# stcodeer/Frequency-wised_All-in-One_Image_Restoration_Model

Hardware: AMD Instinct MI355X
Metric: training images/sec @128x128 (higher is better)
Workload: dtype bf16; 1 GPU; BASELINE configs[1]: Uformer encoder+decoder (all_3_bands, L=3, freq MSA), denoise sigma=25, 128x128, phase-2 train step (fwd+bwd+Adam, DropPath on); per_gpu_batch=16, global_batch=16, parallelism=dp1, hip_graph=True

## Files before the change

frequency-wised_all-in-one_image_restoration_model_amd/csrc/fw_norm.hip:

```cpp
#include "fw_common.h"
#include <stdlib.h>

namespace {

constexpr int NVMAX = 4;

template <int G> FW_DEV float group_sum(float v) {
#pragma unroll
    for (int o = G / 2; o > 0; o >>= 1) v += __shfl_xor(v, o, 64);
    return v;
}

template <typename T> struct RawV;
template <> struct RawV<float> {
    f32x4 v;
    FW_MEM void load(const float* p) { v = *reinterpret_cast<const f32x4*>(p); }
    FW_MEM void unpack(float* f) const { f[0] = v[0]; f[1] = v[1]; f[2] = v[2]; f[3] = v[3]; }
};
template <> struct RawV<bf16raw> {
    uint2 v;
    FW_MEM void load(const bf16raw* p) { v = *reinterpret_cast<const uint2*>(p); }
    FW_MEM void unpack(float* f) const {
        f[0] = __uint_as_float(v.x << 16); f[1] = __uint_as_float(v.x & 0xffff0000u);
        f[2] = __uint_as_float(v.y << 16); f[3] = __uint_as_float(v.y & 0xffff0000u);
// ... 47 lines not shown
            s += v[u][t][0] + v[u][t][1] + v[u][t][2] + v[u][t][3];
        }
        const float mu = group_sum<G>(s) * invc;
        float q = 0.f;
#pragma unroll
        for (int t = 0; t < NV; ++t) {
            if (gl + G * t < nv) {
#pragma unroll
                for (int e = 0; e < 4; ++e) { const float d = v[u][t][e] - mu; q += d * d; }
            }
        }
        const float rs = rsqrtf(group_sum<G>(q) * invc + eps);
        if (row >= rows) continue;
        if (gl == 0) { mean[row] = mu; rstd[row] = rs; }
#pragma unroll
        for (int t = 0; t < NV; ++t) {
            const int c4 = gl + G * t;
            if (c4 < nv) {
                float o[4];
#pragma unroll
                for (int e = 0; e < 4; ++e) o[e] = (v[u][t][e] - mu) * rs * gam[t][e] + bet[t][e];
                if (MOD) {
#pragma unroll
                    for (int e = 0; e < 4; ++e) o[e] += mv[u][t][e];
                }
                T* yp = y + row * ldy + c4 * 4;
                if (sizeof(T) == 4) *reinterpret_cast<f32x4*>(yp) = f32x4{o[0], o[1], o[2], o[3]};
                else *reinterpret_cast<uint2*>(yp) = make_uint2(pack_bf2(o[0], o[1]), pack_bf2(o[2], o[3]));
            }
        }
    }
}

template <typename T, int G, int NV, int U>
__global__ __launch_bounds__(256) void ln_bwd_kernel(const T* __restrict__ dy, long lddy, const float* __restrict__ x, long ldx,
                                                     const float* __restrict__ gamma, const float* __restrict__ mean,
                                                     const float* __restrict__ rstd, const float* __restrict__ dres, long lddres,
                                                     float* __restrict__ dx, long lddx, float* __restrict__ partial,
                                                     long pstride, int rows, int C, T* __restrict__ twin, long ldtw,
                                                     const float* __restrict__ twscale, int tw_rows_per_scale) {
    constexpr int RPB = 256 / G;
    const int gl = threadIdx.x % G, gr = threadIdx.x / G;
    const int nv = C >> 2;
    const float invc = 1.0f / C;
    f32x4 gam[NV], dg[NV], db[NV];
    bool cok[NV];
#pragma unroll
    for (int t = 0; t < NV; ++t) {
        const int c4 = gl + G * t;
        cok[t] = c4 < nv;
        gam[t] = cok[t] ? *reinterpret_cast<const f32x4*>(gamma + c4 * 4) : f32x4{0.f, 0.f, 0.f, 0.f};
        dg[t] = f32x4{0.f, 0.f, 0.f, 0.f};
        db[t] = f32x4{0.f, 0.f, 0.f, 0.f};
    }
    for (long r0 = (long)blockIdx.x * RPB * U; r0 < rows; r0 += (long)gridDim.x * RPB * U) {
        f32x4 xv[U][NV], rr[U][NV];
        RawV<T> dr[U][NV];
        float mu[U], rs[U];
#pragma unroll
        for (int u = 0; u < U; ++u) {
            const long row = r0 + u * RPB + gr;
            const long rc = row < rows ? row : rows - 1;
            mu[u] = mean[rc]; rs[u] = rstd[rc];
#pragma unroll
            for (int t = 0; t < NV; ++t) {
                const int cc = (cok[t] ? gl + G * t : nv - 1) * 4;
                xv[u][t] = *reinterpret_cast<const f32x4*>(x + rc * ldx + cc);
                dr[u][t].load(dy + rc * lddy + cc);
                if (dres) rr[u][t] = *reinterpret_cast<const f32x4*>(dres + rc * lddres + cc);
            }
        }
#pragma unroll
        for (int u = 0; u < U; ++u) {
            const long row = r0 + u * RPB + gr;
            const bool live = row < rows;
            f32x4 xh[NV], g[NV];
            float s1 = 0.f, s2 = 0.f;
#pragma unroll
            for (int t = 0; t < NV; ++t) {
                float d[4];
                dr[u][t].unpack(d);
                const bool ok = live && cok[t];
#pragma unroll
                for (int e = 0; e < 4; ++e) {
                    const float de = ok ? d[e] : 0.f;
                    xh[t][e] = ok ? (xv[u][t][e] - mu[u]) * rs[u] : 0.f;
                    g[t][e] = de * gam[t][e];
                    dg[t][e] += de * xh[t][e];
                    db[t][e] += de;
                    s1 += g[t][e];
                    s2 += g[t][e] * xh[t][e];
                }
            }
            s1 = group_sum<G>(s1) * invc;
            s2 = group_sum<G>(s2) * invc;
            if (!live) continue;
            const float sc = (twin && twscale) ? twscale[row / tw_rows_per_scale] : 1.0f;
#pragma unroll
            for (int t = 0; t < NV; ++t) {
                if (!cok[t]) continue;
                const int c4 = gl + G * t;
                f32x4 o;
#pragma unroll
                for (int e = 0; e < 4; ++e) o[e] = rs[u] * (g[t][e] - s1 - xh[t][e] * s2);
                if (dres) o += rr[u][t];
                *reinterpret_cast<f32x4*>(dx + row * lddx + c4 * 4) = o;
                if (twin) {
                    T* tp = twin + row * ldtw + c4 * 4;
                    if (sizeof(T) == 4) *reinterpret_cast<f32x4*>(tp) = o * sc;
                    else *reinterpret_cast<uint2*>(tp) = make_uint2(pack_bf2(o[0] * sc, o[1] * sc), pack_bf2(o[2] * sc, o[3] * sc));
                }
            }
        }
    }
    __shared__ float red[2][1024];
    for (int i = threadIdx.x; i < 2048; i += 256) (&red[0][0])[i] = 0.f;
    __syncthreads();
#pragma unroll
    for (int t = 0; t < NV; ++t) {
        const int c4 = gl + G * t;
        if (c4 < nv) {
#pragma unroll
            for (int e = 0; e < 4; ++e) {
                atomicAdd(&red[0][c4 * 4 + e], dg[t][e]);
                atomicAdd(&red[1][c4 * 4 + e], db[t][e]);
            }
        }
    }
    __syncthreads();
    float* pp = partial + (long)blockIdx.x * pstride;
    const int Cp = (int)(pstride >> 1);
    for (int c = threadIdx.x; c < Cp; c += 256) {
        pp[c] = c < C ? red[0][c] : 0.f;
        pp[Cp + c] = c < C ? red[1][c] : 0.f;
    }
}

template <typename T, int G, int NV, int U>
int ln_fwd_launch(const float* x, long ldx, const float* g, const float* b, void* y, long ldy, float* mean,
                  float* rstd, int rows, int C, float eps, hipStream_t st) {
    const int rpb = 256 / G * U;
    hipLaunchKernelGGL((ln_fwd_kernel<T, G, NV, U>), dim3(fw_cdiv(rows, rpb)), dim3(256), 0, st, x, ldx, g, b, (T*)y, ldy,
                       mean, rstd, rows, C, eps, (const float*)nullptr, 1, 1, 0);
    FW_LAUNCH_RET();
}
template <typename T, int G, int NV, int U>
int ln_mod_fwd_launch(const float* x, long ldx, const float* g, const float* b, const float* mod, void* y, long ldy, float* mean,
                      float* rstd, int rows, int C, int H, int W, int shift, float eps, hipStream_t st) {
    const int rpb = 256 / G * U;
    hipLaunchKernelGGL((ln_fwd_kernel<T, G, NV, U, true>), dim3(fw_cdiv(rows, rpb)), dim3(256), 0, st, x, ldx, g, b, (T*)y, ldy,
                       mean, rstd, rows, C, eps, mod, H, W, shift);
    FW_LAUNCH_RET();
}
static inline int ln_group(int C) { return C <= 32 ? 8 : (C <= 64 ? 16 : (C <= 128 ? 32 : 64)); }
static inline int ln_rows_per_step(int C) { return C <= 256 ? 4 : (C <= 512 ? 2 : 1); }
static inline int ln_bwd_grid(int rows, int C) {
    const int cap = C > 256 ? 256 : (C > 128 ? 512 : 1024);
    return min(fw_cdiv(rows, 256 / ln_group(C) * ln_rows_per_step(C)), cap);
}

template <typename T, int G, int NV, int U>
int ln_bwd_launch(const void* dy, long lddy, const float* x, long ldx, const float* g, const float* mean,
                  const float* rstd, const float* dres, long lddres, float* dx, long lddx, float* partial, long pstride,
                  int rows, int C, void* twin, long ldtw, const float* twscale, int twrps, hipStream_t st) {
    hipLaunchKernelGGL((ln_bwd_kernel<T, G, NV, U>), dim3(ln_bwd_grid(rows, C)), dim3(256), 0, st, (const T*)dy, lddy, x, ldx, g, mean, rstd,
                       dres, lddres, dx, lddx, partial, pstride, rows, C, (T*)twin, ldtw, twscale, twrps);
    FW_LAUNCH_RET();
}

template <typename T, int E> struct ModV;
template <> struct ModV<float, 4> {
    f32x4 v;
    FW_MEM void load(const float* p) { v = *reinterpret_cast<const f32x4*>(p); }
    FW_MEM void add(float* a) const { a[0] += v[0]; a[1] += v[1]; a[2] += v[2]; a[3] += v[3]; }
};
template <> struct ModV<bf16raw, 4> {
    RawV<bf16raw> r;
    FW_MEM void load(const bf16raw* p) { r.load(p); }
    FW_MEM void add(float* a) const { float f[4]; r.unpack(f); a[0] += f[0]; a[1] += f[1]; a[2] += f[2]; a[3] += f[3]; }
};
template <> struct ModV<bf16raw, 8> {
    uint4 v;
    FW_MEM void load(const bf16raw* p) { v = *reinterpret_cast<const uint4*>(p); }
    FW_MEM void add(float* a) const {
        const unsigned w[4] = {v.x, v.y, v.z, v.w};
#pragma unroll
        for (int i = 0; i < 4; ++i) { a[2 * i] += __uint_as_float(w[i] << 16); a[2 * i + 1] += __uint_as_float(w[i] & 0xffff0000u); }
    }
};

constexpr int MOD_LD = 8;

template <typename T, int E, int CL>
__global__ __launch_bounds__(256) void mod_bwd_kernel(const T* __restrict__ dy, long lddy, float* __restrict__ partial, int n, int per,
                                                      int C, int W, int shift) {
    constexpr int TG = 32 / CL;
    const int cl = threadIdx.x % CL, tg = threadIdx.x / CL % TG, xq = threadIdx.x / 32;
    const int yq = blockIdx.y, z = blockIdx.z;
    const int col = (blockIdx.x * CL + cl) * E;
    const bool cok = col < C;
// ... 48 lines not shown
    hipLaunchKernelGGL((mod_bwd_kernel<T, E, CL>), dim3(fw_cdiv(nvr, CL), 8, nz), dim3(256), 0, st, (const T*)dy, lddy, partial, n, \
                       per, C, W, shift)
    if (nvr <= 8) MOD_B(8);
    else if (nvr <= 16) MOD_B(16);
    else MOD_B(32);
#undef MOD_B
    FW_LAUNCH_RET();
}

#define LN_DISPATCH(FN, T, ...)                                    \
    (C <= 32 ? FN<T, 8, 1, 4>(__VA_ARGS__)                         \
     : C <= 64 ? FN<T, 16, 1, 4>(__VA_ARGS__)                      \
     : C <= 128 ? FN<T, 32, 1, 4>(__VA_ARGS__)                     \
     : C <= 256 ? FN<T, 64, 1, 4>(__VA_ARGS__)                     \
     : C <= 512 ? FN<T, 64, 2, 2>(__VA_ARGS__)                     \
                : FN<T, 64, 4, 1>(__VA_ARGS__))

}

extern "C" int fw_layernorm_fwd(int dtype, const float* x, long ldx, const float* gamma, const float* beta, void* y,
                                long ldy, float* mean, float* rstd, int rows, int C, float eps, void* stream) {
    FW_CHECK_ARG(rows > 0 && C > 0 && C % 4 == 0 && C <= 1024 && ldx % 4 == 0 && ldy % 4 == 0);
    FW_CHECK_ARG(x && gamma && beta && y && mean && rstd);
    hipStream_t st = (hipStream_t)stream;
#define LN_F(T) LN_DISPATCH(ln_fwd_launch, T, x, ldx, gamma, beta, y, ldy, mean, rstd, rows, C, eps, st)
    return dtype == FW_DT_BF16 ? LN_F(bf16raw) : LN_F(float);
#undef LN_F
}

extern "C" int fw_layernorm_bwd_blocks(int rows, int C) { return ln_bwd_grid(rows, C); }

extern "C" int fw_slab_reduce(const float* slab, int nz, long n, long zstride, float* dst, int accumulate, float* dst2, long off2, long n2,
                              void* stream);
extern "C" int fw_layernorm_bwd2(int dtype, const void* dy, long lddy, const float* x, long ldx, const float* gamma,
                                 const float* mean, const float* rstd, const float* dres, long lddres, float* dx,
                                 long lddx, float* dgamma, float* dbeta, float* partial, int rows, int C, void* twin, long ldtw,
                                 const float* twscale, int tw_rows_per_scale, void* stream) {
    FW_CHECK_ARG(rows > 0 && C > 0 && C % 4 == 0 && C <= 1024 && ldx % 4 == 0 && lddy % 4 == 0 && lddx % 4 == 0);
    FW_CHECK_ARG(dy && x && gamma && mean && rstd && dx && partial && ((dgamma && dbeta) || (!dgamma && !dbeta)));
    FW_CHECK_ARG(!twin || (ldtw % 4 == 0 && (!twscale || tw_rows_per_scale > 0)));
    hipStream_t st = (hipStream_t)stream;
    const long pstride = 2L * C;
#define LN_B(T)                                                                                                          \
    LN_DISPATCH(ln_bwd_launch, T, dy, lddy, x, ldx, gamma, mean, rstd, dres, lddres, dx, lddx, partial, pstride, rows, C, twin, \
                ldtw, twscale, tw_rows_per_scale, st)
    const int rc = dtype == FW_DT_BF16 ? LN_B(bf16raw) : LN_B(float);
#undef LN_B
    if (rc || !dgamma) return rc;
    return fw_slab_reduce(partial, ln_bwd_grid(rows, C), C, pstride, dgamma, 1, dbeta, C, C, stream);
}

extern "C" int fw_layernorm_bwd(int dtype, const void* dy, long lddy, const float* x, long ldx, const float* gamma,
                                const float* mean, const float* rstd, const float* dres, long lddres, float* dx,
                                long lddx, float* dgamma, float* dbeta, float* partial, int rows, int C, void* stream) {
    return fw_layernorm_bwd2(dtype, dy, lddy, x, ldx, gamma, mean, rstd, dres, lddres, dx, lddx, dgamma, dbeta, partial, rows, C,
                             nullptr, 0, nullptr, 1, stream);
}

extern "C" int fw_layernorm_mod_fwd(int dtype, const float* x, long ldx, const float* gamma, const float* beta, const float* mod, void* y,
                                    long ldy, float* mean, float* rstd, int rows, int C, int H, int W, int shift, float eps, void* stream) {
    FW_CHECK_ARG(rows > 0 && C > 0 && C % 4 == 0 && C <= 1024 && ldx % 4 == 0 && ldy % 4 == 0);
    FW_CHECK_ARG(x && gamma && beta && mod && y && mean && rstd && ((uintptr_t)mod & 15) == 0);
    FW_CHECK_ARG(H > 0 && W > 0 && H % 8 == 0 && W % 8 == 0 && rows % ((long)H * W) == 0 && shift >= 0 && shift < 8);
    hipStream_t st = (hipStream_t)stream;
#define LN_F(T) LN_DISPATCH(ln_mod_fwd_launch, T, x, ldx, gamma, beta, mod, y, ldy, mean, rstd, rows, C, H, W, shift, eps, st)
    return dtype == FW_DT_BF16 ? LN_F(bf16raw) : LN_F(float);
#undef LN_F
}

extern "C" int fw_modulator_bwd_blocks(int rows, int C) { return mod_bwd_slices(rows, C); }

extern "C" int fw_modulator_bwd(int dtype, const void* dy, long lddy, float* dmod, float* partial, int rows, int C, int H, int W, int shift,
                                void* stream) {
    FW_CHECK_ARG(rows > 0 && C > 0 && C % 4 == 0 && C <= 1024 && lddy % 4 == 0 && lddy >= C);
    FW_CHECK_ARG(dy && partial && ((uintptr_t)partial & 15) == 0);
    FW_CHECK_ARG(H > 0 && W > 0 && H % 8 == 0 && W % 8 == 0 && rows % ((long)H * W) == 0 && shift >= 0 && shift < 8);
    hipStream_t st = (hipStream_t)stream;
    int rc;
    if (dtype != FW_DT_BF16) {
        FW_CHECK_ARG(((uintptr_t)dy & 15) == 0);
        rc = mod_bwd_launch<float, 4>(dy, lddy, partial, rows, C, W, shift, st);
    } else if (C % 8 == 0 && lddy % 8 == 0 && ((uintptr_t)dy & 15) == 0) {
// ... 9 lines not shown
```

frequency-wised_all-in-one_image_restoration_model_amd/fwair/functional.py:

```python
import weakref

import torch

from . import ops
from .lib import call, dt


class config:
    compute_dtype = torch.float32
    shadow_epoch = 0
    direct_grads = False


def act_empty(rows, cols, dtype, device):
    ld = (cols + 7) // 8 * 8
    return torch.empty((rows, ld), dtype=dtype, device=device)[:, :cols]


def aligned(t):
    if t.stride(1) == 1 and (t.stride(0) * t.element_size()) % 16 == 0 and t.data_ptr() % 16 == 0:
        return t
    out = act_empty(t.shape[0], t.shape[1], t.dtype, t.device)
    out.copy_(t)
    return out


_shadow = {}


def shadow(param, kind='plain'):
    dtype = config.compute_dtype
    p = param.detach()
    fs = getattr(param, '_fw_shadow', None)
    if fs is not None and kind == 'plain' and fs.dtype == dtype:
        return fs
    if kind == 'plain' and dtype == torch.float32:
        w = p.reshape(p.shape[0], -1)
        if (w.stride(0) * 4) % 16 == 0:
            return w
    slot = _shadow.get(id(param))
    ent = slot[1] if slot is not None and slot[0]() is param else None
    key = (kind, dtype)
    stamp = (param._version, config.shadow_epoch, p.data_ptr())
    if ent is not None and key in ent and ent[key][0] == stamp:
# ... 123 lines not shown
                _retired_tables.append(_refresh_tables[which])
            _refresh_tables[which] = cached
        call('fw_permute3_multi', cached[1], cached[2], cached[3], cached[4])
    for ent, key, fresh, out, recipe in stamps:
        ent[key] = (fresh, out, recipe)


def _zeros(shape, device):
    return torch.zeros(shape, dtype=torch.float32, device=device)


def _grad_target(param, shape=None):
    if config.direct_grads and param is not None and param.grad is not None:
        g = param.grad
        return (g if shape is None else g.view(shape)), None
    z = _zeros(param.shape if shape is None else shape, param.device)
    return z, z


def _wgrad(g, x, n, k, m, weight, bias=None):
    dw, rw = _grad_target(weight, (n, k))
    db, rb = _grad_target(bias) if bias is not None else (None, None)
    direct = rw is None and rb is None
    ops.wgrad(g, x, n, k, m, dw, db, defer=direct)
    return (rw.view_as(weight) if rw is not None else None), rb


def _bgrad(g, bias):
    db, rb = _grad_target(bias)
    ops.colsum(g, db)
    return rb


class LayerNormFn(torch.autograd.Function):
    @staticmethod
    def forward(ctx, x, gamma, beta):
        rows, C = x.shape
        y = act_empty(rows, C, config.compute_dtype, x.device)
        mean = torch.empty(rows, dtype=torch.float32, device=x.device)
        rstd = torch.empty(rows, dtype=torch.float32, device=x.device)
        call('fw_layernorm_fwd', dt(y.dtype), x, x.stride(0), gamma, beta, y, y.stride(0), mean, rstd, rows, C, 1e-5)
        ctx.save_for_backward(x, gamma, mean, rstd)
        ctx.beta = beta
        return y

    @staticmethod
    def backward(ctx, dy):
        x, gamma, mean, rstd = ctx.saved_tensors
        dy = aligned(dy)
        beta = ctx.beta
        dg, rg = _grad_target(gamma)
        db, rb = _grad_target(beta)
        dx = ops.layernorm_bwd(dy, x, gamma, mean, rstd, dg, db, defer=rg is None and rb is None)
        return dx, rg, rb


class LinearFn(torch.autograd.Function):

    @staticmethod
    def forward(ctx, x, weight, bias, residual, rowscale, rows_per_scale, x_pre, gelu_out, out_f32, fuse=None):
        ctx.set_materialize_grads(False)
        M, K = x.shape
        N = weight.shape[0]
        if fuse is not None and not gelu_out:
            y, g = fuse['y'], None
        elif fuse is not None:
            y, g = _leff_fused_forward(x, weight, bias, fuse)
        else:
            w = shadow(weight)
            if residual is not None or out_f32:
                y = torch.empty((M, N), dtype=torch.float32, device=x.device)
            else:
                y = act_empty(M, N, x.dtype, x.device)
            g = act_empty(M, N, x.dtype, x.device) if gelu_out else None
            ops.gemm(x, w, M, N, K, out=y, bias=bias, rowscale=rowscale, rows_per_scale=rows_per_scale, residual=residual,
                     out_gelu=g)
        ctx.save_for_backward(x, weight, rowscale, x_pre)
        ctx.bias = bias
        ctx.cfg = (rows_per_scale, residual is not None)
        if gelu_out:
            ctx.mark_non_differentiable(g)
            return y, g
        return y

    @staticmethod
    def backward(ctx, dy, *_):
        if dy is None:
            return (None,) * 10
        x, weight, rowscale, x_pre = ctx.saved_tensors
        rows_per_scale, has_res = ctx.cfg
        bias = ctx.bias
        M, K = x.shape
        N = weight.shape[0]
        tw = getattr(dy, '_fw_twin', None)
        if (tw is not None and tw[0].dtype == x.dtype and tw[0].shape == (M, N) and tw[2] == rows_per_scale
                and (tw[1] is rowscale or (tw[1] is not None and rowscale is not None and tw[1].data_ptr() == rowscale.data_ptr()))):
            g = tw[0]
        elif dy.dtype == torch.float32 and x.dtype != torch.float32 or rowscale is not None:
            g = act_empty(M, N, x.dtype, x.device)
            call('fw_cast_rows', dt(x.dtype), dy, dy.stride(0), g, g.stride(0), M, N, rowscale, rows_per_scale)
        else:
            g = aligned(dy)
        dw, db = _wgrad(g, x, N, K, M, weight, bias)
        dx = dpre = None
        if ctx.needs_input_grad[0] or (x_pre is not None and ctx.needs_input_grad[6]):
            d = act_empty(M, K, x.dtype, x.device)
            ops.dgrad(g, shadow(weight), M, K, N, d, act=2 if x_pre is not None else 0, aux=x_pre)
            if x_pre is not None:
                dpre = d
            else:
                dx = d
        return dx, dw, db, (dy if has_res else None), None, None, dpre, None, None, None


def _leff_fused_forward(xn, w1, b1, fuse):
    M, C = xn.shape
    B, H, W = fuse['geo']
    C4 = w1.shape[0]
    h1, g1 = act_empty(M, C4, xn.dtype, xn.device), act_empty(M, C4, xn.dtype, xn.device)
    h2, g2 = act_empty(M, C4, xn.dtype, xn.device), act_empty(M, C4, xn.dtype, xn.device)
    y = torch.empty((M, C), dtype=torch.float32, device=xn.device)
    res, rs = fuse['residual'], fuse['rowscale']
    call('fw_leff_fwd', xn, xn.stride(0), shadow(w1, 'leff1'), b1, shadow(fuse['wd'], 'dw9'), fuse['bd'], shadow(fuse['w2'], 'leff2'), fuse['b2'],
         res, res.stride(0), rs, fuse['rows_per_scale'], y, y.stride(0), h1, g1, h2, g2, h1.stride(0), B, H, W, C)
    fuse['h2'], fuse['g2'], fuse['y'] = h2, g2, y
    return h1, g1


class LnResFn(torch.autograd.Function):

    @staticmethod
    def forward(ctx, x, gamma, beta):
        ctx.set_materialize_grads(False)
        ctx.rs_hint = getattr(x, '_fw_rs', None)
        rows, C = x.shape
        y = act_empty(rows, C, config.compute_dtype, x.device)
        mean = torch.empty(rows, dtype=torch.float32, device=x.device)
        rstd = torch.empty(rows, dtype=torch.float32, device=x.device)
        call('fw_layernorm_fwd', dt(y.dtype), x, x.stride(0), gamma, beta, y, y.stride(0), mean, rstd, rows, C, 1e-5)
        ctx.save_for_backward(x, gamma, mean, rstd)
        ctx.beta = beta
        return x.view_as(x), y

    @staticmethod
    def backward(ctx, dres, dy):
        x, gamma, mean, rstd = ctx.saved_tensors
        dg, rg = _grad_target(gamma)
        db, rb = _grad_target(ctx.beta)
        if dy is None:
            return dres, None, None
        dy = aligned(dy)
        twin = None
        if ctx.rs_hint is not None:
            twin = act_empty(x.shape[0], x.shape[1], dy.dtype, x.device)
        rs, rps = ctx.rs_hint if ctx.rs_hint is not None else (None, 1)
        dx = ops.layernorm_bwd(dy, x, gamma, mean, rstd, dg, db, dres=dres, defer=rg is None and rb is None, twin=twin, twscale=rs,
                               tw_rows_per_scale=rps)
        if twin is not None:
            dx._fw_twin = (twin, rs, rps)
        return dx, rg, rb


class LnResModFn(torch.autograd.Function):

    @staticmethod
    def forward(ctx, x, gamma, beta, mod, geo):
        ctx.set_materialize_grads(False)
        ctx.rs_hint = getattr(x, '_fw_rs', None)
        rows, C = x.shape
        y = act_empty(rows, C, config.compute_dtype, x.device)
        mean, rstd = ops.layernorm_mod_fwd(x, gamma, beta, mod, geo[0], geo[1], geo[2], y)
        ctx.save_for_backward(x, gamma, mean, rstd)
        ctx.beta, ctx.mod, ctx.geo = beta, mod, geo
        return x.view_as(x), y

    @staticmethod
    def backward(ctx, dres, dy):
        x, gamma, mean, rstd = ctx.saved_tensors
        dg, rg = _grad_target(gamma)
        db, rb = _grad_target(ctx.beta)
        if dy is None:
            return dres, None, None, None, None
        dm, rm = _grad_target(ctx.mod)
        dy = aligned(dy)
# ... 10 lines not shown


def linear(x, weight, bias=None, residual=None, rowscale=None, rows_per_scale=1, x_pre=None, gelu_out=False, out_f32=False, fuse=None):
    y = LinearFn.apply(x, weight, bias, residual, rowscale, rows_per_scale, x_pre, gelu_out, out_f32, fuse)
    if residual is not None and y.requires_grad and (x.dtype != torch.float32 or rowscale is not None):
        y._fw_rs = (rowscale, rows_per_scale)
    return y


class QKVFn(torch.autograd.Function):

    @staticmethod
    def forward(ctx, x, wq, bq, wkv, bkv, fused):
        M, K = x.shape
        C = wq.shape[0]
        Cp = (C + 7) // 8 * 8
        buf = act_empty(M, Cp + 2 * C, x.dtype, x.device)
        if fused is not None and Cp == C:
            w3 = fused['sw'] if x.dtype == torch.bfloat16 and 'sw' in fused else (fused['w'] if x.dtype == torch.float32 else None)
        else:
            w3 = None
        ctx.cat = None
        if w3 is not None:
            ops.gemm(x, w3, M, 3 * C, K, out=buf[:, :3 * C], bias=fused['b'])
        elif Cp != C and bq is not None and bkv is not None:
            wc, bc = shadow_qkv(wq, bq, wkv, bkv)
            ops.gemm(x, wc, M, Cp + 2 * C, K, out=buf, bias=bc)
            ctx.cat = wc
        else:
            ops.gemm(x, shadow(wq), M, C, K, out=buf[:, :C], bias=bq)
            ops.gemm(x, shadow(wkv), M, 2 * C, K, out=buf[:, Cp:], bias=bkv)
        ctx.save_for_backward(x, wq, wkv)
        ctx.bq, ctx.bkv = bq, bkv
        ctx.fused = (fused, w3)
        return buf

    @staticmethod
    def backward(ctx, dbuf):
        x, wq, wkv = ctx.saved_tensors
        M, K = x.shape
        C = wq.shape[0]
        Cp = (C + 7) // 8 * 8
        dbuf = aligned(dbuf)
        fused, w3 = ctx.fused
        dx = act_empty(M, K, x.dtype, x.device)
        if w3 is not None and config.direct_grads and 'gw' in fused:
            ops.wgrad(dbuf[:, :3 * C], x, 3 * C, K, M, fused['gw'], fused['gb'], defer=True)
            ops.dgrad(dbuf[:, :3 * C], w3, M, K, 3 * C, dx)
            return dx, None, None, None, None, None
        dq, dkv = dbuf[:, :C], dbuf[:, Cp:]
        dwq, dbq = _wgrad(dq, x, C, K, M, wq, ctx.bq)
        dwkv, dbkv = _wgrad(dkv, x, 2 * C, K, M, wkv, ctx.bkv)
        if ctx.cat is not None and getattr(dbuf, '_fw_zero_pad', False):
            ops.gemm(dbuf, ctx.cat, M, K, Cp + 2 * C, w_trans=True, out=dx)
            return dx, dwq, dbq, dwkv, dbkv, None
        tmp = torch.empty((M, K), dtype=torch.float32, device=x.device)
        ops.gemm(dq, shadow(wq), M, K, C, w_trans=True, out=tmp)
        ops.gemm(dkv, shadow(wkv), M, K, 2 * C, w_trans=True, out=dx, residual=tmp)
        return dx, dwq, dbq, dwkv, dbkv, None


class WindowAttnFn(torch.autograd.Function):

    @staticmethod
    def forward(ctx, qkv, tables, coef, geo, tparam, dcoef_to):
        ctx.side = (tparam, dcoef_to)
        C, B, H, W, heads, L, mode, shift, lfs = geo
        D = C // heads
        Cp = (C + 7) // 8 * 8
        rows = qkv.shape[0]
        nkt = 1 if mode == 0 else L - 1
        out = act_empty(rows, C, qkv.dtype, qkv.device)
        lse = torch.empty((B * (H // 8) * (W // 8) * L * heads, 64), dtype=torch.float32, device=qkv.device)
        tab = ops._lfs.device_table(qkv.dtype, qkv.device) if lfs == 2 else None
        call('fw_attn_fwd', dt(qkv.dtype), D, nkt, lfs, qkv, qkv[:, Cp:], qkv[:, Cp + C:], qkv.stride(0), out, out.stride(0),
             lse, tables, coef, tab, B, H, W, heads, L, mode, shift, float(D) ** -0.5)
        ctx.save_for_backward(qkv, tables, coef, out, lse)
        ctx.geo = geo
        return out

    @staticmethod
# ... 530 lines not shown
```

frequency-wised_all-in-one_image_restoration_model_amd/fwair/ops.py:

```python
import bisect

import torch

from . import lfs as _lfs
from .lib import call, dt, lib


def _ld(t):
    assert t.dim() == 2 and t.stride(1) == 1, 'expect a row-major 2-D view'
    return t.stride(0)


def empty(rows, cols, dtype, device):
    return torch.empty((rows, cols), dtype=dtype, device=device)


def gemm(x, w, M, N, K, *, x_trans=False, w_trans=False, x_op=0, w_op=0, out=None, out_dtype=None, bias=None,
         act=0, slope=0.0, aux=None, rowscale=None, rows_per_scale=1, residual=None, accumulate=False, splitk=1,
         alpha=1.0, out_gelu=None, xsum=None, c_zstride=0, xsum_zstride=0):
    assert x.dtype == w.dtype
    if out is None:
        out = torch.empty((M, N), dtype=out_dtype or x.dtype, device=x.device)
    if accumulate:
        _note_write(out)
# ... 284 lines not shown
    host[:nprob * 16].view(nprob, 16).copy_(torch.tensor(rows, dtype=torch.int64))
    it32 = torch.tensor(items, dtype=torch.int32)
    host[nprob * 16:].view(torch.int32).view(total, 4).copy_(it32)
    table = torch.empty(host.shape, dtype=torch.int64, device=dev)
    table.copy_(host, non_blocking=True)
    probs = torch.empty(nprob * lib().fw_wgrad_group_prob_bytes(), dtype=torch.uint8, device=dev)
    _group_fire(table, probs, nprob, total, tile)
    if not torch.cuda.is_current_stream_capturing():
        for slot in _host_ring:
            if slot[0].data_ptr() == host.data_ptr():
                slot[1].record()


def wgrad(g, x, n, k, m, dw, db=None, defer=False):
    if defer and _in_backward() and _groupable(g, x, n, k, m, dw, db):
        _register_flush()
        _pending_w.append((g, x, n, k, m, dw, db))
        return
    _note_write(dw)
    _note_write(db)
    sk = pick_splitk(n, k, m, g.dtype)
    if sk == 1:
        gemm(g, x, n, k, m, x_trans=True, w_trans=True, out=dw, accumulate=True, xsum=db)
        return
    nk = (n * k + 3) // 4 * 4
    S = nk + (n + 3) // 4 * 4
    slab = torch.empty((sk, S), dtype=torch.float32, device=g.device)
    cview = slab[0, :n * k].view(n, k)
    xs = slab[0, nk:] if db is not None else None
    gemm(g, x, n, k, m, x_trans=True, w_trans=True, out=cview, splitk=sk, xsum=xs, c_zstride=S, xsum_zstride=S if db is not None else 0)
    slab_reduce(slab, sk, n * k, S, dw, db, nk, n, defer=defer)


def dgrad(g, w, M, K, N, out, act=0, aux=None):
    tiles = ((M + 127) // 128) * ((K + 127) // 128)
    sk = min(512 // max(tiles, 1), N // _DGRAD_SPLIT_ROWS) if (act == 0 and tiles < 200) else 1
    if sk <= 1:
        gemm(g, w, M, K, N, w_trans=True, out=out, act=act, aux=aux)
        return
    S = (M * K + 3) // 4 * 4
    slab = torch.empty((sk, S), dtype=torch.float32, device=g.device)
    gemm(g, w, M, K, N, w_trans=True, out=slab[0, :M * K].view(M, K), splitk=sk, c_zstride=S)
    direct = out.dtype == torch.float32 and out.is_contiguous()
    tmp = out if direct else torch.empty((M, K), dtype=torch.float32, device=g.device)
    call('fw_slab_reduce', slab, sk, M * K, S, tmp, 0, None, 0, 0)
    if not direct:
        call('fw_cast_rows', dt(out.dtype), tmp, K, out, _ld(out), M, K, None, 1)


def layernorm_fwd(x, gamma, beta, out_dtype, eps=1e-5):
    rows, C = x.shape
    y = torch.empty((rows, C), dtype=out_dtype, device=x.device)
    mean = torch.empty(rows, dtype=torch.float32, device=x.device)
    rstd = torch.empty(rows, dtype=torch.float32, device=x.device)
    call('fw_layernorm_fwd', dt(out_dtype), x, _ld(x), gamma, beta, y, _ld(y), mean, rstd, rows, C, eps)
    return y, mean, rstd


def layernorm_bwd(dy, x, gamma, mean, rstd, dgamma, dbeta, dres=None, defer=False, twin=None, twscale=None, tw_rows_per_scale=1):
    rows, C = x.shape
    dx = torch.empty((rows, C), dtype=torch.float32, device=x.device)
    nblk = lib().fw_layernorm_bwd_blocks(rows, C)
    partial = torch.empty((nblk, 2 * C), dtype=torch.float32, device=x.device)
    call('fw_layernorm_bwd2', dt(dy.dtype), dy, _ld(dy), x, _ld(x), gamma, mean, rstd, dres,
         _ld(dres) if dres is not None else 0, dx, _ld(dx), None, None, partial, rows, C,
         twin, _ld(twin) if twin is not None else 0, twscale, tw_rows_per_scale)
    slab_reduce(partial, nblk, C, 2 * C, dgamma, dbeta, C, C, defer=defer)
    return dx


def layernorm_mod_fwd(x, gamma, beta, mod, H, W, shift, y, eps=1e-5):
    rows, C = x.shape
    mean = torch.empty(rows, dtype=torch.float32, device=x.device)
    rstd = torch.empty(rows, dtype=torch.float32, device=x.device)
    call('fw_layernorm_mod_fwd', dt(y.dtype), x, _ld(x), gamma, beta, mod, y, _ld(y), mean, rstd, rows, C, H, W, shift, eps)
    return mean, rstd


def modulator_bwd(dy, dmod, H, W, shift, defer=False):
    rows, C = dy.shape
    nz = lib().fw_modulator_bwd_blocks(rows, C)
    partial = torch.empty((nz, 64 * C), dtype=torch.float32, device=dy.device)
    deferred = defer and _in_backward()
    if not deferred:
        _note_write(dmod)
    call('fw_modulator_bwd', dt(dy.dtype), dy, _ld(dy), None if deferred else dmod, partial, rows, C, H, W, shift)
    if deferred:
        slab_reduce(partial, nz, 64 * C, 64 * C, dmod, defer=True)


def attn_fwd(qkv, C, B, H, W, heads, L, mode, shift, bias, coef=None, lfs=0):
    rows = qkv.shape[0]
    D = C // heads
    nkt = 1 if mode == 0 else L - 1
    out = torch.empty((rows, C), dtype=qkv.dtype, device=qkv.device)
    nitems = B * (H // 8) * (W // 8) * L * heads
    lse = torch.empty((nitems, 64), dtype=torch.float32, device=qkv.device)
# ... 97 lines not shown
```

include/fwair.h:

```cpp
#ifndef FWAIR_H
#define FWAIR_H
#ifdef __cplusplus
extern "C" {
#endif

int fw_gemm(int dtype, const void* X, long ldx, int x_trans, int x_op, const void* W, long ldw, int w_trans, int w_op,
            void* C, long ldc, int out_f32, int accumulate, int M, int N, int K, float alpha, const float* bias, int act,
            float slope, const void* aux, long ldaux, const float* rowscale, int rows_per_scale, const float* residual,
            long ldr, int splitk, void* C2, long ldc2, float* xsum, long c_zstride, long xsum_zstride, void* stream);
int fw_gemm_last_kernel(char* buf, int n);

int fw_wgrad_group_prob_bytes(void);
int fw_wgrad_group(const void* tab, void* probs, int nprob, const void* items, int nitems, int tile, void* stream);

int fw_slab_reduce(const float* slab, int nz, long n, long zstride, float* dst, int accumulate, float* dst2, long off2, long n2,
                   void* stream);
int fw_slab_reduce_multi(const void* tab, const void* prefix, int num, long total_blocks, void* stream);

int fw_layernorm_fwd(int dtype, const float* x, long ldx, const float* gamma, const float* beta, void* y, long ldy,
                     float* mean, float* rstd, int rows, int C, float eps, void* stream);
int fw_layernorm_bwd_blocks(int rows, int C);
int fw_layernorm_bwd(int dtype, const void* dy, long lddy, const float* x, long ldx, const float* gamma, const float* mean,
                     const float* rstd, const float* dres, long lddres, float* dx, long lddx, float* dgamma, float* dbeta,
                     float* partial, int rows, int C, void* stream);
int fw_layernorm_bwd2(int dtype, const void* dy, long lddy, const float* x, long ldx, const float* gamma, const float* mean,
                      const float* rstd, const float* dres, long lddres, float* dx, long lddx, float* dgamma, float* dbeta,
                      float* partial, int rows, int C, void* twin, long ldtw, const float* twscale, int tw_rows_per_scale,
                      void* stream);

int fw_layernorm_mod_fwd(int dtype, const float* x, long ldx, const float* gamma, const float* beta, const float* mod, void* y,
                         long ldy, float* mean, float* rstd, int rows, int C, int H, int W, int shift, float eps, void* stream);
int fw_modulator_bwd_blocks(int rows, int C);
int fw_modulator_bwd(int dtype, const void* dy, long lddy, float* dmod, float* partial, int rows, int C, int H, int W, int shift,
                     void* stream);

int fw_attn_lfs_table_elems(void);
int fw_attn_fwd(int dtype, int D, int nkt, int lfs, const void* q, const void* k, const void* v, long ld, void* out, long ldo,
                float* lse, const float* bias, const float* coef, const void* lfs_tab, int B, int H, int W, int heads, int L,
                int mode, int shift, float scale, void* stream);
int fw_attn_bwd(int dtype, int D, int nkt, int lfs, const void* q, const void* k, const void* v, long ld, const void* out,
                long ldo, const void* dout, long lddo, const float* lse, const float* bias, const float* coef,
                const void* lfs_tab, void* dq, void* dk, void* dv, void* dk2, void* dv2, long ldd, float* dbias,
                float* dcoef, int B, int H, int W, int heads, int L, int mode, int shift, float scale, int dq_pad, void* stream);
int fw_attn_chunks(int dtype, int D, int nkt, int lfs, int backward, int nwin, int heads, int L);

int fw_dwconv_fwd(int dtype, const void* in, long ld1, int in_gelu, const float* w, const float* bias, void* h2, void* g2, long ld2, int B,
                  int H, int W, int C, void* stream);
int fw_dwconv_bwd(int dtype, const void* dh2, long ldg, const void* g1, const void* h1, long ld1, const float* w, void* dh1,
                  long ldo, float* dw, float* dbias, int B, int H, int W, int C, void* stream);

int fw_im2col4(int dtype, const float* x, long ldx, void* col, int B, int H, int W, int C, void* stream);
int fw_col2im4(int dtype, const void* dcol, float* dx, long lddx, const float* dres, long ldr, int B, int H, int W, int C,
               void* stream);
int fw_pixel_shuffle(int dtype, const void* g, const float* bias, float* out, long ldo, int B, int H, int W, int Cout,
                     void* stream);
int fw_pixel_unshuffle(int dtype, const float* dout, long ldo, void* dg, int B, int H, int W, int Cout, void* stream);
int fw_colsum(int x_dtype, const void* x, long ldx, float* out, long rows, int cols, void* stream);

int fw_inproj_fwd(const float* img, const float* w, const float* bias, float* out, long ldo, int B, int H, int W, int C,
                  float slope, void* stream);
int fw_inproj_bwd(const float* img, const float* out, long ldo, const float* dy, long ldy, float* dw, float* db, int B, int H,
// ... 146 lines not shown
```

Measured before the change: 347.9 images/sec.

## Fuse split-K dgrad slab reduction into LayerNorm backward and widen LN bwd blocks

When a Linear/QKV dgrad uses split-K and its input comes straight from a LayerNorm, the slab is no longer reduced and cast. It is attached to the gradient tensor, and the LayerNorm backward kernel sums the slab partials in place of loading dy. This drops a separate slab-reduce pass, an optional cast kernel, and a full round-trip of the dx buffer. The change also replaces the shared-memory atomicAdd reduction of dgamma/dbeta with per-row slots summed serially, and uses 512-thread blocks for C>128 with a changed grid cap. In exchange the backward relies on autograd metadata passing through intact, which needs runtime checks and a config flag.

```diff
diff --git a/frequency-wised_all-in-one_image_restoration_model_amd/csrc/fw_norm.hip b/frequency-wised_all-in-one_image_restoration_model_amd/csrc/fw_norm.hip
--- a/frequency-wised_all-in-one_image_restoration_model_amd/csrc/fw_norm.hip
+++ b/frequency-wised_all-in-one_image_restoration_model_amd/csrc/fw_norm.hip
@@ -103,14 +103,46 @@
     }
 }
 
-template <typename T, int G, int NV, int U>
-__global__ __launch_bounds__(256) void ln_bwd_kernel(const T* __restrict__ dy, long lddy, const float* __restrict__ x, long ldx,
+FW_DEV f32x4 slab_dy_sum(const float* __restrict__ p, int nz, long zs) {
+    f32x4 s[4];
+#pragma unroll
+    for (int j = 0; j < 4; ++j) s[j] = f32x4{0.f, 0.f, 0.f, 0.f};
+    if (nz <= 4) {
+        s[0] += *reinterpret_cast<const f32x4*>(p);
+        if (nz > 1) s[1] += *reinterpret_cast<const f32x4*>(p + zs);
+        if (nz > 2) s[2] += *reinterpret_cast<const f32x4*>(p + 2 * zs);
+        if (nz > 3) s[3] += *reinterpret_cast<const f32x4*>(p + 3 * zs);
+    } else {
+#pragma unroll
+        for (int j = 0; j < 4; ++j) {
+            int z = j;
+            for (; z + 12 < nz; z += 16) {
+                const f32x4 a0 = *reinterpret_cast<const f32x4*>(p + (long)z * zs);
+                const f32x4 a1 = *reinterpret_cast<const f32x4*>(p + (long)(z + 4) * zs);
+                const f32x4 a2 = *reinterpret_cast<const f32x4*>(p + (long)(z + 8) * zs);
+                const f32x4 a3 = *reinterpret_cast<const f32x4*>(p + (long)(z + 12) * zs);
+                s[j] += (a0 + a1) + (a2 + a3);
+            }
+            for (; z < nz; z += 4) s[j] += *reinterpret_cast<const f32x4*>(p + (long)z * zs);
+        }
+    }
+    return s[0] + ((s[1] + s[2]) + s[3]);
+}
+template <typename T> FW_DEV void raw_from_sum(RawV<T>& r, const f32x4& s);
+template <> FW_SPEC void raw_from_sum<float>(RawV<float>& r, const f32x4& s) { r.v = s; }
+template <> FW_SPEC void raw_from_sum<bf16raw>(RawV<bf16raw>& r, const f32x4& s) {
+    r.v = make_uint2(pack_bf2(s[0], s[1]), pack_bf2(s[2], s[3]));
+}
+
+template <typename T, int G, int NV, int U, int TPB, bool SLAB>
+__global__ __launch_bounds__(TPB) void ln_bwd_kernel(const T* __restrict__ dy, long lddy, const float* __restrict__ slab, int nz, long zstride,
+                                                     const float* __restrict__ x, long ldx,
                                                      const float* __restrict__ gamma, const float* __restrict__ mean,
                                                      const float* __restrict__ rstd, const float* __restrict__ dres, long lddres,
                                                      float* __restrict__ dx, long lddx, float* __restrict__ partial,
                                                      long pstride, int rows, int C, T* __restrict__ twin, long ldtw,
                                                      const float* __restrict__ twscale, int tw_rows_per_scale) {
-    constexpr int RPB = 256 / G;
+    constexpr int RPB = TPB / G;
     const int gl = threadIdx.x % G, gr = threadIdx.x / G;
     const int nv = C >> 2;
     const float invc = 1.0f / C;
@@ -137,8 +169,20 @@
             for (int t = 0; t < NV; ++t) {
                 const int cc = (cok[t] ? gl + G * t : nv - 1) * 4;
                 xv[u][t] = *reinterpret_cast<const f32x4*>(x + rc * ldx + cc);
-                dr[u][t].load(dy + rc * lddy + cc);
+                if (!SLAB) dr[u][t].load(dy + rc * lddy + cc);
                 if (dres) rr[u][t] = *reinterpret_cast<const f32x4*>(dres + rc * lddres + cc);
+            }
+        }
+        if (SLAB) {
+#pragma unroll
+            for (int u = 0; u < U; ++u) {
+                const long row = r0 + u * RPB + gr;
+                const long rc = row < rows ? row : rows - 1;
+#pragma unroll
+                for (int t = 0; t < NV; ++t) {
+                    const int cc = (cok[t] ? gl + G * t : nv - 1) * 4;
+                    raw_from_sum<T>(dr[u][t], slab_dy_sum(slab + rc * C + cc, nz, zstride));
+                }
             }
         }
 #pragma unroll
@@ -184,26 +228,26 @@
             }
         }
     }
-    __shared__ float red[2][1024];
-    for (int i = threadIdx.x; i < 2048; i += 256) (&red[0][0])[i] = 0.f;
-    __syncthreads();
+    constexpr int COLS = NV * 4 * G;
+    __shared__ float red[RPB][2][COLS];
 #pragma unroll
     for (int t = 0; t < NV; ++t) {
         const int c4 = gl + G * t;
-        if (c4 < nv) {
-#pragma unroll
-            for (int e = 0; e < 4; ++e) {
-                atomicAdd(&red[0][c4 * 4 + e], dg[t][e]);
-                atomicAdd(&red[1][c4 * 4 + e], db[t][e]);
-            }
-        }
+        *reinterpret_cast<f32x4*>(&red[gr][0][c4 * 4]) = dg[t];
+        *reinterpret_cast<f32x4*>(&red[gr][1][c4 * 4]) = db[t];
     }
     __syncthreads();
     float* pp = partial + (long)blockIdx.x * pstride;
     const int Cp = (int)(pstride >> 1);
-    for (int c = threadIdx.x; c < Cp; c += 256) {
-        pp[c] = c < C ? red[0][c] : 0.f;
-        pp[Cp + c] = c < C ? red[1][c] : 0.f;
+    for (int c = threadIdx.x; c < Cp; c += TPB) {
+        float a = 0.f, b = 0.f;
+        if (c < C) {
+            a = red[0][0][c]; b = red[0][1][c];
+#pragma unroll
+            for (int k = 1; k < RPB; ++k) { a += red[k][0][c]; b += red[k][1][c]; }
+        }
+        pp[c] = a;
+        pp[Cp + c] = b;
     }
 }
 
@@ -225,18 +269,39 @@
 }
 static inline int ln_group(int C) { return C <= 32 ? 8 : (C <= 64 ? 16 : (C <= 128 ? 32 : 64)); }
 static inline int ln_rows_per_step(int C) { return C <= 256 ? 4 : (C <= 512 ? 2 : 1); }
+constexpr int LN_BWD_WIDE_TPB = 512;
 static inline int ln_bwd_grid(int rows, int C) {
-    const int cap = C > 256 ? 256 : (C > 128 ? 512 : 1024);
-    return min(fw_cdiv(rows, 256 / ln_group(C) * ln_rows_per_step(C)), cap);
-}
-
-template <typename T, int G, int NV, int U>
-int ln_bwd_launch(const void* dy, long lddy, const float* x, long ldx, const float* g, const float* mean,
-                  const float* rstd, const float* dres, long lddres, float* dx, long lddx, float* partial, long pstride,
-                  int rows, int C, void* twin, long ldtw, const float* twscale, int twrps, hipStream_t st) {
-    hipLaunchKernelGGL((ln_bwd_kernel<T, G, NV, U>), dim3(ln_bwd_grid(rows, C)), dim3(256), 0, st, (const T*)dy, lddy, x, ldx, g, mean, rstd,
-                       dres, lddres, dx, lddx, partial, pstride, rows, C, (T*)twin, ldtw, twscale, twrps);
+    const int tpb = C > 128 ? LN_BWD_WIDE_TPB : 256;
+    const int cap = C > 512 ? 256 : (C > 128 ? 512 : 1024);
+    return min(fw_cdiv(rows, tpb / ln_group(C) * ln_rows_per_step(C)), cap);
+}
+
+struct LnBwdArgs {
+    const void* dy; long lddy; const float* slab; int nz; long zstride;
+    const float* x; long ldx; const float* g; const float* mean; const float* rstd; const float* dres; long lddres;
+    float* dx; long lddx; float* partial; long pstride; int rows, C; void* twin; long ldtw; const float* twscale; int twrps;
+};
+template <typename T, int G, int NV, int U, int TPB>
+int ln_bwd_launch(const LnBwdArgs& a, hipStream_t st) {
+    const dim3 grid(ln_bwd_grid(a.rows, a.C)), block(TPB);
+#define LN_BK(SLAB)                                                                                                                  \
+    hipLaunchKernelGGL((ln_bwd_kernel<T, G, NV, U, TPB, SLAB>), grid, block, 0, st, (const T*)a.dy, a.lddy, a.slab, a.nz, a.zstride, a.x, \
+                       a.ldx, a.g, a.mean, a.rstd, a.dres, a.lddres, a.dx, a.lddx, a.partial, a.pstride, a.rows, a.C, (T*)a.twin, a.ldtw, \
+                       a.twscale, a.twrps)
+    if (a.slab) LN_BK(true);
+    else LN_BK(false);
+#undef LN_BK
     FW_LAUNCH_RET();
+}
+template <typename T>
+int ln_bwd_dispatch(const LnBwdArgs& a, hipStream_t st) {
+    const int C = a.C;
+    return C <= 32    ? ln_bwd_launch<T, 8, 1, 4, 256>(a, st)
+           : C <= 64  ? ln_bwd_launch<T, 16, 1, 4, 256>(a, st)
+           : C <= 128 ? ln_bwd_launch<T, 32, 1, 4, 256>(a, st)
+           : C <= 256 ? ln_bwd_launch<T, 64, 1, 4, LN_BWD_WIDE_TPB>(a, st)
+           : C <= 512 ? ln_bwd_launch<T, 64, 2, 2, LN_BWD_WIDE_TPB>(a, st)
+                      : ln_bwd_launch<T, 64, 4, 1, LN_BWD_WIDE_TPB>(a, st);
 }
 
 template <typename T, int E> struct ModV;
@@ -351,22 +416,31 @@
 
 extern "C" int fw_slab_reduce(const float* slab, int nz, long n, long zstride, float* dst, int accumulate, float* dst2, long off2, long n2,
                               void* stream);
+extern "C" int fw_layernorm_bwd_slab(int dtype, const void* dy, long lddy, const float* dy_slab, int nz, long zstride, const float* x, long ldx,
+                                     const float* gamma, const float* mean, const float* rstd, const float* dres, long lddres, float* dx,
+                                     long lddx, float* dgamma, float* dbeta, float* partial, int rows, int C, void* twin, long ldtw,
+                                     const float* twscale, int tw_rows_per_scale, void* stream) {
+    FW_CHECK_ARG(rows > 0 && C > 0 && C % 4 == 0 && C <= 1024 && ldx % 4 == 0 && lddx % 4 == 0);
+    FW_CHECK_ARG(x && gamma && mean && rstd && dx && partial && ((dgamma && dbeta) || (!dgamma && !dbeta)));
+    FW_CHECK_ARG(!twin || (ldtw % 4 == 0 && (!twscale || tw_rows_per_scale > 0)));
+    if (dy_slab) FW_CHECK_ARG(nz > 0 && zstride % 4 == 0 && zstride >= (long)rows * C && ((uintptr_t)dy_slab & 15) == 0);
+    else FW_CHECK_ARG(dy && lddy % 4 == 0);
+    hipStream_t st = (hipStream_t)stream;
+    const long pstride = 2L * C;
+    const LnBwdArgs a{dy, lddy, dy_slab, nz, zstride, x, ldx, gamma, mean, rstd, dres, lddres, dx, lddx, partial, pstride, rows, C,
+                      twin, ldtw, twscale, tw_rows_per_scale};
+    const int rc = dtype == FW_DT_BF16 ? ln_bwd_dispatch<bf16raw>(a, st) : ln_bwd_dispatch<float>(a, st);
+    if (rc || !dgamma) return rc;
+    return fw_slab_reduce(partial, ln_bwd_grid(rows, C), C, pstride, dgamma, 1, dbeta, C, C, stream);
+}
+
 extern "C" int fw_layernorm_bwd2(int dtype, const void* dy, long lddy, const float* x, long ldx, const float* gamma,
                                  const float* mean, const float* rstd, const float* dres, long lddres, float* dx,
                                  long lddx, float* dgamma, float* dbeta, float* partial, int rows, int C, void* twin, long ldtw,
                                  const float* twscale, int tw_rows_per_scale, void* stream) {
-    FW_CHECK_ARG(rows > 0 && C > 0 && C % 4 == 0 && C <= 1024 && ldx % 4 == 0 && lddy % 4 == 0 && lddx % 4 == 0);
-    FW_CHECK_ARG(dy && x && gamma && mean && rstd && dx && partial && ((dgamma && dbeta) || (!dgamma && !dbeta)));
-    FW_CHECK_ARG(!twin || (ldtw % 4 == 0 && (!twscale || tw_rows_per_scale > 0)));
-    hipStream_t st = (hipStream_t)stream;
-    const long pstride = 2L * C;
-#define LN_B(T)                                                                                                          \
-    LN_DISPATCH(ln_bwd_launch, T, dy, lddy, x, ldx, gamma, mean, rstd, dres, lddres, dx, lddx, partial, pstride, rows, C, twin, \
-                ldtw, twscale, tw_rows_per_scale, st)
-    const int rc = dtype == FW_DT_BF16 ? LN_B(bf16raw) : LN_B(float);
-#undef LN_B
-    if (rc || !dgamma) return rc;
-    return fw_slab_reduce(partial, ln_bwd_grid(rows, C), C, pstride, dgamma, 1, dbeta, C, C, stream);
+    FW_CHECK_ARG(dy);
+    return fw_layernorm_bwd_slab(dtype, dy, lddy, nullptr, 0, 0, x, ldx, gamma, mean, rstd, dres, lddres, dx, lddx, dgamma, dbeta, partial,
+                                 rows, C, twin, ldtw, twscale, tw_rows_per_scale, stream);
 }
 
 extern "C" int fw_layernorm_bwd(int dtype, const void* dy, long lddy, const float* x, long ldx, const float* gamma,
diff --git a/frequency-wised_all-in-one_image_restoration_model_amd/fwair/functional.py b/frequency-wised_all-in-one_image_restoration_model_amd/fwair/functional.py
--- a/frequency-wised_all-in-one_image_restoration_model_amd/fwair/functional.py
+++ b/frequency-wised_all-in-one_image_restoration_model_amd/fwair/functional.py
@@ -10,6 +10,7 @@
     compute_dtype = torch.float32
     shadow_epoch = 0
     direct_grads = False
+    lazy_dgrad = True
 
 
 def act_empty(rows, cols, dtype, device):
@@ -199,6 +200,33 @@
     return rb
 
 
+def _ln_publish(ctx, y):
+    ctx.ln_cell = y._fw_ln = [0, False]
+
+
+def _ln_consume(ctx, x):
+    cell = getattr(x, '_fw_ln', None) if ctx.needs_input_grad[0] else None
+    if cell is not None:
+        cell[0] += 1
+    ctx.ln_cell = cell
+
+
+def _ln_may_be_lazy(ctx):
+    return config.lazy_dgrad and ctx.ln_cell is not None and ctx.ln_cell[0] == 1
+
+
+def _ln_take(ctx, dy):
+    cell = ctx.ln_cell
+    went, cell[1] = cell[1], False
+    if dy is not None and getattr(dy, '_fw_slab', None) is not None:
+        return dy
+    if went:
+        raise RuntimeError('fwair: a Linear left its input gradient in a split-K slab for this LayerNorm, but the gradient that arrived '
+                           'does not carry it (the LayerNorm output has a consumer that is not a LinearFn / QKVFn, or the gradient was '
+                           'copied on the way); set functional.config.lazy_dgrad = False for such a graph')
+    return aligned(dy) if dy is not None else None
+
+
 class LayerNormFn(torch.autograd.Function):
     @staticmethod
     def forward(ctx, x, gamma, beta):
@@ -209,12 +237,13 @@
         call('fw_layernorm_fwd', dt(y.dtype), x, x.stride(0), gamma, beta, y, y.stride(0), mean, rstd, rows, C, 1e-5)
         ctx.save_for_backward(x, gamma, mean, rstd)
         ctx.beta = beta
+        _ln_publish(ctx, y)
         return y
 
     @staticmethod
     def backward(ctx, dy):
         x, gamma, mean, rstd = ctx.saved_tensors
-        dy = aligned(dy)
+        dy = _ln_take(ctx, dy)
         beta = ctx.beta
         dg, rg = _grad_target(gamma)
         db, rb = _grad_target(beta)
@@ -245,6 +274,7 @@
         ctx.save_for_backward(x, weight, rowscale, x_pre)
         ctx.bias = bias
         ctx.cfg = (rows_per_scale, residual is not None)
+        _ln_consume(ctx, x)
         if gelu_out:
             ctx.mark_non_differentiable(g)
             return y, g
@@ -272,7 +302,9 @@
         dx = dpre = None
         if ctx.needs_input_grad[0] or (x_pre is not None and ctx.needs_input_grad[6]):
             d = act_empty(M, K, x.dtype, x.device)
-            ops.dgrad(g, shadow(weight), M, K, N, d, act=2 if x_pre is not None else 0, aux=x_pre)
+            if ops.dgrad(g, shadow(weight), M, K, N, d, act=2 if x_pre is not None else 0, aux=x_pre,
+                         lazy=x_pre is None and _ln_may_be_lazy(ctx)):
+                ctx.ln_cell[1] = True
             if x_pre is not None:
                 dpre = d
             else:
@@ -307,6 +339,7 @@
         call('fw_layernorm_fwd', dt(y.dtype), x, x.stride(0), gamma, beta, y, y.stride(0), mean, rstd, rows, C, 1e-5)
         ctx.save_for_backward(x, gamma, mean, rstd)
         ctx.beta = beta
+        _ln_publish(ctx, y)
         return x.view_as(x), y
 
     @staticmethod
@@ -314,9 +347,9 @@
         x, gamma, mean, rstd = ctx.saved_tensors
         dg, rg = _grad_target(gamma)
         db, rb = _grad_target(ctx.beta)
+        dy = _ln_take(ctx, dy)
         if dy is None:
             return dres, None, None
-        dy = aligned(dy)
         twin = None
         if ctx.rs_hint is not None:
             twin = act_empty(x.shape[0], x.shape[1], dy.dtype, x.device)
@@ -393,6 +426,7 @@
             ops.gemm(x, shadow(wkv), M, 2 * C, K, out=buf[:, Cp:], bias=bkv)
         ctx.save_for_backward(x, wq, wkv)
         ctx.bq, ctx.bkv = bq, bkv
+        _ln_consume(ctx, x)
         ctx.fused = (fused, w3)
         return buf
 
@@ -407,7 +441,8 @@
         dx = act_empty(M, K, x.dtype, x.device)
         if w3 is not None and config.direct_grads and 'gw' in fused:
             ops.wgrad(dbuf[:, :3 * C], x, 3 * C, K, M, fused['gw'], fused['gb'], defer=True)
-            ops.dgrad(dbuf[:, :3 * C], w3, M, K, 3 * C, dx)
+            if ops.dgrad(dbuf[:, :3 * C], w3, M, K, 3 * C, dx, lazy=_ln_may_be_lazy(ctx)):
+                ctx.ln_cell[1] = True
             return dx, None, None, None, None, None
         dq, dkv = dbuf[:, :C], dbuf[:, Cp:]
         dwq, dbq = _wgrad(dq, x, C, K, M, wq, ctx.bq)
diff --git a/frequency-wised_all-in-one_image_restoration_model_amd/fwair/ops.py b/frequency-wised_all-in-one_image_restoration_model_amd/fwair/ops.py
--- a/frequency-wised_all-in-one_image_restoration_model_amd/fwair/ops.py
+++ b/frequency-wised_all-in-one_image_restoration_model_amd/fwair/ops.py
@@ -340,20 +340,24 @@
     slab_reduce(slab, sk, n * k, S, dw, db, nk, n, defer=defer)
 
 
-def dgrad(g, w, M, K, N, out, act=0, aux=None):
+def dgrad(g, w, M, K, N, out, act=0, aux=None, lazy=False):
     tiles = ((M + 127) // 128) * ((K + 127) // 128)
     sk = min(512 // max(tiles, 1), N // _DGRAD_SPLIT_ROWS) if (act == 0 and tiles < 200) else 1
     if sk <= 1:
         gemm(g, w, M, K, N, w_trans=True, out=out, act=act, aux=aux)
-        return
+        return False
     S = (M * K + 3) // 4 * 4
     slab = torch.empty((sk, S), dtype=torch.float32, device=g.device)
     gemm(g, w, M, K, N, w_trans=True, out=slab[0, :M * K].view(M, K), splitk=sk, c_zstride=S)
+    if lazy:
+        out._fw_slab = (slab, sk, S)
+        return True
     direct = out.dtype == torch.float32 and out.is_contiguous()
     tmp = out if direct else torch.empty((M, K), dtype=torch.float32, device=g.device)
     call('fw_slab_reduce', slab, sk, M * K, S, tmp, 0, None, 0, 0)
     if not direct:
         call('fw_cast_rows', dt(out.dtype), tmp, K, out, _ld(out), M, K, None, 1)
+    return False
 
 
 def layernorm_fwd(x, gamma, beta, out_dtype, eps=1e-5):
@@ -370,7 +374,10 @@
     dx = torch.empty((rows, C), dtype=torch.float32, device=x.device)
     nblk = lib().fw_layernorm_bwd_blocks(rows, C)
     partial = torch.empty((nblk, 2 * C), dtype=torch.float32, device=x.device)
-    call('fw_layernorm_bwd2', dt(dy.dtype), dy, _ld(dy), x, _ld(x), gamma, mean, rstd, dres,
+    slab, sk, S = getattr(dy, '_fw_slab', None) or (None, 0, 0)
+    if slab is not None and tuple(dy.shape) != (rows, C):
+        raise RuntimeError(f'fwair: layernorm_bwd: slab gradient of shape {tuple(dy.shape)} for rows of shape {(rows, C)}')
+    call('fw_layernorm_bwd_slab', dt(dy.dtype), None if slab is not None else dy, _ld(dy), slab, sk, S, x, _ld(x), gamma, mean, rstd, dres,
          _ld(dres) if dres is not None else 0, dx, _ld(dx), None, None, partial, rows, C,
          twin, _ld(twin) if twin is not None else 0, twscale, tw_rows_per_scale)
     slab_reduce(partial, nblk, C, 2 * C, dgamma, dbeta, C, C, defer=defer)
diff --git a/include/fwair.h b/include/fwair.h
--- a/include/fwair.h
+++ b/include/fwair.h
@@ -27,6 +27,10 @@
                       const float* rstd, const float* dres, long lddres, float* dx, long lddx, float* dgamma, float* dbeta,
                       float* partial, int rows, int C, void* twin, long ldtw, const float* twscale, int tw_rows_per_scale,
                       void* stream);
+int fw_layernorm_bwd_slab(int dtype, const void* dy, long lddy, const float* dy_slab, int nz, long zstride, const float* x, long ldx,
+                          const float* gamma, const float* mean, const float* rstd, const float* dres, long lddres, float* dx,
+                          long lddx, float* dgamma, float* dbeta, float* partial, int rows, int C, void* twin, long ldtw,
+                          const float* twscale, int tw_rows_per_scale, void* stream);
 
 int fw_layernorm_mod_fwd(int dtype, const float* x, long ldx, const float* gamma, const float* beta, const float* mod, void* y,
                          long ldy, float* mean, float* rstd, int rows, int C, int H, int W, int shift, float eps, void* stream);
```

Measured after the change: 356.5 images/sec (median of 6 runs). +2.5%, better.
